# Alvin-Zeng/DRN

Measured on AMD Instinct MI355X. Metric: clips/sec fwd+bwd (BxT=256x4096 C3D feats), higher is better.
Workload: dtype bf16; 1 GPU; Charades-STA-shaped C3D features, T=256, D=4096, batch 32/GPU, stage-1 losses; step = fwd+bwd+grad all-reduce+clip(0.5)+Adam; global_batch=32, T=256, D=4096, parallelism=dp1

## Files before the change

drn_amd/csrc/api.hip:

```cpp
#include <stdarg.h>
#include "common.h"
#include "../../include/drn_hip.h"

static thread_local char g_err[512] = "";

void drn_set_error(const char* fmt, ...) {
  va_list ap;
  va_start(ap, fmt);
  vsnprintf(g_err, sizeof(g_err), fmt, ap);
  va_end(ap);
}

extern "C" int drn_abi_version(void) {
  drn_clear_status(); return DRN_ABI_VERSION; }
extern "C" const char* drn_last_error(void) { return g_err; }

static int g_tune[16] = {4096, 1, 256, 0, 0, 0, 0, 0, 1, 1, 0, 16, 160, 512, 2048, 1};
int drn_tuning(int key) { return g_tune[key]; }
extern "C" int drn_tune(const char* key, int value) {
  drn_clear_status();
  if (key && !strcmp(key, "tn3_minrows")) { g_tune[DRN_TUNE_TN3_MINROWS] = value; return DRN_OK; }
  if (key && !strcmp(key, "tn_fused")) { g_tune[DRN_TUNE_TN_FUSED] = value; return DRN_OK; }
  if (key && !strcmp(key, "nt_w4c")) { g_tune[DRN_TUNE_NT_W4C] = value; return DRN_OK; }
  if (key && !strcmp(key, "nt_w4")) { g_tune[DRN_TUNE_NT_W4] = value; return DRN_OK; }
  if (key && !strcmp(key, "nt_deep")) { g_tune[DRN_TUNE_NT_DEEP] = value; return DRN_OK; }
  if (key && !strcmp(key, "nt_w4h")) { g_tune[DRN_TUNE_NT_W4H] = value; return DRN_OK; }
  if (key && !strcmp(key, "w4h_tapil")) { g_tune[DRN_TUNE_W4H_TAPIL] = value; return DRN_OK; }
  if (key && !strcmp(key, "w4h_halo")) { g_tune[DRN_TUNE_W4H_HALO] = value; return DRN_OK; }
  if (key && !strcmp(key, "bn1_maxwg")) { g_tune[DRN_TUNE_BN1_MAXWG] = value; return DRN_OK; }
  if (key && !strcmp(key, "nt_deep2")) { g_tune[DRN_TUNE_NT_DEEP2] = value; return DRN_OK; }
  if (key && !strcmp(key, "nt_deep_ks")) { g_tune[DRN_TUNE_NT_DEEP_KS] = value; return DRN_OK; }
  if (key && !strncmp(key, "exp", 3) && key[3] >= '0' && key[3] <= '4' && !key[4]) { g_tune[DRN_TUNE_EXP0 + (key[3] - '0')] = value; return DRN_OK; }
  drn_set_error("drn_tune: unknown key %s", key ? key : "(null)");
  return DRN_ERR_ARG;
}
```

drn_amd/csrc/common.h:

```cpp
#pragma once
#include <hip/hip_runtime.h>
#include <stdint.h>
#include <stdio.h>
#include <string.h>

#define DRN_OK 0
#define DRN_ERR_ARG (-1)
#define DRN_ERR_LAUNCH (-2)
#define DRN_ERR_UNSUPPORTED (-3)

#define DRN_F32 0
#define DRN_BF16 1

typedef __bf16 bf16_t;
typedef __bf16 bf16x8 __attribute__((ext_vector_type(8)));
typedef __bf16 bf16x4 __attribute__((ext_vector_type(4)));
typedef short s16x4 __attribute__((ext_vector_type(4)));
typedef float f32x4 __attribute__((ext_vector_type(4)));
typedef float f32x2 __attribute__((ext_vector_type(2)));

template <typename T>
__device__ __forceinline__ T* as_global(T* p) {
  typedef __attribute__((address_space(1))) T* g_t;
  g_t g = (g_t)p;
  asm("" : "+s"(g));
  return (T*)g;
}
template <typename T>
__device__ __forceinline__ T* as_global_v(T* p) {
  typedef __attribute__((address_space(1))) T* g_t;
  g_t g = (g_t)p;
  asm("" : "+v"(g));
  return (T*)g;
}


void drn_set_error(const char* fmt, ...);

#define DRN_CHECK_ARG(cond, ...)          \
  do {                                    \
    if (!(cond)) {                        \
      drn_set_error(__VA_ARGS__);         \
      return DRN_ERR_ARG;                 \
    }                                     \
  } while (0)

static inline void drn_clear_status() { (void)hipGetLastError(); }

static inline int drn_launch_status(const char* what) {
  hipError_t e = hipGetLastError();
  if (e != hipSuccess) {
    drn_set_error("%s: launch failed: %s", what, hipGetErrorString(e));
    return DRN_ERR_LAUNCH;
  }
  return DRN_OK;
}

static inline int cdiv(int a, int b) { return (a + b - 1) / b; }

int drn_tuning(int key);
#define DRN_XCHG_CONFIRM 0x20000
#define DRN_XCHG_READBACK 0x40000
#define DRN_XCHG_NONE 0x80000
#define DRN_TUNE_TN3_MINROWS 0
#define DRN_TUNE_TN_FUSED 1
#define DRN_TUNE_EXP0 3
#define DRN_TUNE_NT_W4C 9
#define DRN_TUNE_NT_W4 8
#define DRN_TUNE_NT_DEEP 2
#define DRN_TUNE_NT_W4H 12
#define DRN_TUNE_BN1_MAXWG 13
#define DRN_TUNE_W4H_TAPIL 14
#define DRN_TUNE_W4H_HALO 15
#define DRN_TUNE_NT_DEEP2 10
#define DRN_TUNE_NT_DEEP_KS 11

static __device__ uint4 g_zero_page[4];

template <typename T> struct DT;
template <> struct DT<float> {
  static __device__ __forceinline__ float ld(const float* p) { return *p; }
  static __device__ __forceinline__ void st(float* p, float v) { *p = v; }
  static __device__ __forceinline__ float round(float v) { return v; }
};
template <> struct DT<bf16_t> {
  static __device__ __forceinline__ float ld(const bf16_t* p) { return (float)*p; }
  static __device__ __forceinline__ void st(bf16_t* p, float v) { *p = (bf16_t)v; }
  static __device__ __forceinline__ float round(float v) { return (float)(bf16_t)v; }
};

__device__ __forceinline__ float wave_sum(float v) {
#pragma unroll
  for (int o = 32; o > 0; o >>= 1) v += __shfl_xor(v, o, 64);
  return v;
}

__device__ __forceinline__ float block_sum(float v, float* sh ) {
  v = wave_sum(v);
  const int w = threadIdx.x >> 6, l = threadIdx.x & 63, nw = blockDim.x >> 6;
  __syncthreads();
  if (l == 0) sh[w] = v;
  __syncthreads();
  if (w == 0) {
    float t = l < nw ? sh[l] : 0.f;
    t = wave_sum(t);
    if (l == 0) sh[16] = t;
  }
  __syncthreads();
  return sh[16];
}
```

drn_amd/csrc/gemm_tn.hip:

```cpp
#include <type_traits>
#include "common.h"
#include "../../include/drn_hip.h"



struct WgradGroup {
  const void* dY;
  const void* X;
  int M, Lout, Lsrc, ldy, ldx;
  int blk_start;
};
struct WgradParams {
  int ngroups;
  WgradGroup g[DRN_MAX_GROUPS];
  int total_blks, blks_per_split;
  int N, Cin, taps, stride, pad;
  int ctiles;
  float* out;
  int direct;
  int w_layout;
  int accumulate;
  int multi;
  int z_start[DRN_MAX_GROUPS + 1], bps[DRN_MAX_GROUPS], gdirect[DRN_MAX_GROUPS];
  int gcin[DRN_MAX_GROUPS];
// ... 237 lines not shown
        if (c >= Cin) continue;
        float v = acc[mi][ni][r];
        if (direct) {
          float* dst = P.w_layout == 0 ? out_ptr + ((long)n * KW + tap * Cin + c)
                                       : out_ptr + ((long)n * KW + (long)c * P.taps + tap);
          if (P.accumulate) v += *dst;
          *dst = v;
        } else {
          out_ptr[((long)split * P.N + n) * KW + tap * Cin + c] = v;
        }
      }
    }
}

__device__ __forceinline__ bf16x8 tr_frag(const char* lo_addr, const char* hi_addr) {
  typedef __attribute__((address_space(3))) s16x4* lp;
  union { struct { s16x4 a, b; } s; bf16x8 v; } u;
  u.s.a = __builtin_amdgcn_ds_read_tr16_b64_v4i16((lp)lo_addr);
  u.s.b = __builtin_amdgcn_ds_read_tr16_b64_v4i16((lp)hi_addr);
  return u.v;
}

template <int NSTG>
__global__ __launch_bounds__(512, 2) void conv_wgrad3_tn_kernel(const WgradParams P) {
  extern __shared__ __attribute__((aligned(16))) char smem[];
  typedef bf16_t T;
  constexpr int R = 64, MI = 4, NI = 2;
  constexpr int IMG = 16384, HALO_B = 512, STAGE_B = 2 * IMG + HALO_B;
  const int tid = threadIdx.x, w = __builtin_amdgcn_readfirstlane(tid >> 6), l = tid & 63;
  const int n0 = blockIdx.x * 128, c0 = blockIdx.y * 128;
  int split = blockIdx.z;
  int blk_lo = split * P.blks_per_split;
  int blk_hi = min(blk_lo + P.blks_per_split, P.total_blks);
  float* out_ptr = P.out;
  int direct = P.direct;
  if (P.multi) {
    int pg = 0;
#pragma unroll
    for (int i = 1; i < DRN_MAX_GROUPS; ++i)
      if (i < P.ngroups && (int)blockIdx.z >= P.z_start[i]) pg = i;
    split = blockIdx.z - P.z_start[pg];
    const int blk_end = pg + 1 < P.ngroups ? P.g[pg + 1].blk_start : P.total_blks;
    blk_lo = P.g[pg].blk_start + split * P.bps[pg];
    blk_hi = min(blk_lo + P.bps[pg], blk_end);
    out_ptr = P.gout[pg];
    direct = P.gdirect[pg];
  }
  const T* zero = (const T*)g_zero_page;

  const int srow = w * 8 + (l >> 3);
  const int scol = (((l & 7) >> 1) ^ ((srow >> 1) & 3)) * 16 + (l & 1) * 8;
  long y_off[2], x_off[2];
#pragma unroll
  for (int j = 0; j < 2; ++j) {
    y_off[j] = n0 + j * 64 + scol < P.N ? n0 + j * 64 + scol : -1;
    x_off[j] = c0 + j * 64 + scol < P.Cin ? c0 + j * 64 + scol : -1;
  }
  const bool is_halo = (w == 0) & (l < 32);
  const int hcol = ((l >> 3) & 1) * 64 + (l & 7) * 8;
  const long xh_off = c0 + hcol < P.Cin ? c0 + hcol : -1;
  const int rowoff[2] = {srow, (l >> 4) ? R : -1};
  int s_blk = blk_lo, s_g = 0;
#pragma unroll
  for (int i = 1; i < DRN_MAX_GROUPS; ++i)
    if (i < P.ngroups && blk_lo >= P.g[i].blk_start) s_g = i;
  int s_seq[2], s_t[2];
  const T* g_Y;
  const T* g_X;
  int g_L, g_nseq, g_ldy, g_ldx, g_next;
  auto locate = [&]() {
    const WgradGroup& G = P.g[s_g];
    g_Y = (const T*)G.dY;
    g_X = (const T*)G.X;
    g_L = G.Lout;
    g_nseq = G.M / G.Lout;
    g_ldy = G.ldy;
    g_ldx = G.ldx;
    g_next = s_g + 1 < P.ngroups ? P.g[s_g + 1].blk_start : 0x7fffffff;
    const int Lp = G.Lout + 1;
    const int pbase = (s_blk - G.blk_start) * R;
#pragma unroll
    for (int j = 0; j < 2; ++j) {
      const int p = pbase + rowoff[j] + Lp;
      const int q = p / Lp;
      s_seq[j] = q - 1;
      s_t[j] = p - q * Lp;
    }
  };
  locate();

  auto row_ptr = [&](const T* base, int m, int ld, long coff, bool ok) -> const T* {
    const unsigned off = __umul24((unsigned)m, (unsigned)ld) + (unsigned)coff;
    const T* p = base + off;
    return ok ? p : zero;
  };
  auto stage_part = [&](int buf, int part) {
    char* Ys = smem + buf * STAGE_B;
    char* Xs = Ys + IMG;
    char* Hs = Xs + IMG;
    const bool live = s_blk < blk_hi;
    const int L = g_L;
    const bool ok = live & ((unsigned)s_seq[0] < (unsigned)g_nseq) & (s_t[0] < L);
    const int m = s_seq[0] * L + s_t[0];
    if (part == 0) glds16(row_ptr(g_Y, m, g_ldy, y_off[0], ok & (y_off[0] >= 0)), Ys + w * 1024);
    if (part == 1) glds16(row_ptr(g_X, m, g_ldx, x_off[0], ok & (x_off[0] >= 0)), Xs + w * 1024);
    if (part == 2) glds16(row_ptr(g_Y, m, g_ldy, y_off[1], ok & (y_off[1] >= 0)), Ys + 8192 + w * 1024);
    if (part == 3) {
      glds16(row_ptr(g_X, m, g_ldx, x_off[1], ok & (x_off[1] >= 0)), Xs + 8192 + w * 1024);
      if (is_halo) {
        const bool okh = live & ((unsigned)s_seq[1] < (unsigned)g_nseq) & (s_t[1] < L) & (xh_off >= 0);
        glds16(row_ptr(g_X, s_seq[1] * L + s_t[1], g_ldx, xh_off, okh), Hs);
      }
    }
    if (part != 4) return;
    ++s_blk;
    if (s_blk >= g_next) {
      ++s_g;
      locate();
    } else {
      const int Lp = L + 1;
      if (Lp > R) {
#pragma unroll
        for (int j = 0; j < 2; ++j) {
          s_t[j] += R;
          const bool wrap = s_t[j] >= Lp;
          s_t[j] -= wrap ? Lp : 0;
          s_seq[j] += wrap ? 1 : 0;
        }
      } else {
#pragma unroll
        for (int j = 0; j < 2; ++j) {
          s_t[j] += R;
          while (s_t[j] >= Lp) {
            s_t[j] -= Lp;
            ++s_seq[j];
          }
        }
      }
    }
  };
  auto stage = [&](int buf) {
#pragma unroll
    for (int part = 0; part < 5; ++part) stage_part(buf, part);
  };

  f32x4 acc[3][MI][NI];
#pragma unroll
  for (int t = 0; t < 3; ++t)
#pragma unroll
    for (int mi = 0; mi < MI; ++mi)
#pragma unroll
      for (int ni = 0; ni < NI; ++ni) acc[t][mi][ni] = (f32x4){0.f, 0.f, 0.f, 0.f};
  const int wr = w >> 2, wc = w & 3;

  const int fr = (l >> 4) * 4 + ((l & 15) >> 2);
  const int fb = (l & 3) * 8;
  int ya[MI], xa[3][NI], x_first[NI], x_last[NI];
#pragma unroll
  for (int mi = 0; mi < MI; ++mi) ya[mi] = wr * 8192 + fr * 128 + ((mi ^ ((fr >> 1) & 3)) * 32) + fb;
#pragma unroll
  for (int ni = 0; ni < NI; ++ni) {
    const int half = wc >> 1, cb = (wc & 1) * 2 + ni;
#pragma unroll
    for (int t = 0; t < 3; ++t) {
      const int rr = fr + t - 1;
      xa[t][ni] = IMG + half * 8192 + rr * 128 + ((cb ^ ((rr >> 1) & 3)) * 32) + fb;
    }
    x_first[ni] = fr == 0 ? 2 * IMG + half * 128 + cb * 32 + fb : xa[0][ni];
    x_last[ni] = fr == 15 ? 2 * IMG + 256 + half * 128 + cb * 32 + fb : xa[2][ni] + 4096 + 2048;
  }

  struct Frags {
    bf16x8 a[MI], b[3][NI];
  };
  auto load_frags = [&](Frags& F, const char* S, auto ks_) {
    constexpr int ks = decltype(ks_)::value;
#pragma unroll
    for (int mi = 0; mi < MI; ++mi) {
      const char* q = S + ya[mi] + ks * 4096;
      F.a[mi] = tr_frag(q, q + 2048);
    }
#pragma unroll
    for (int ni = 0; ni < NI; ++ni) {
      const char* q0 = S + xa[0][ni] + ks * 4096;
      const char* q1 = S + xa[1][ni] + ks * 4096;
      const char* q2 = S + xa[2][ni] + ks * 4096;
      F.b[1][ni] = tr_frag(q1, q1 + 2048);
      F.b[0][ni] = tr_frag(ks == 0 ? S + x_first[ni] : q0, q0 + 2048);
      F.b[2][ni] = tr_frag(q2, ks == 1 ? S + x_last[ni] : q2 + 2048);
    }
  };
  auto mfma_frags = [&](const Frags& F, int mi0) {
#pragma unroll
    for (int t = 0; t < 3; ++t)
#pragma unroll
      for (int mi = 0; mi < 2; ++mi)
#pragma unroll
        for (int ni = 0; ni < NI; ++ni)
          acc[t][mi0 + mi][ni] = __builtin_amdgcn_mfma_f32_16x16x32_bf16(F.a[mi0 + mi], F.b[t][ni], acc[t][mi0 + mi][ni], 0, 0, 0);
  };
  typedef std::integral_constant<int, 0> K0;
  typedef std::integral_constant<int, 1> K1;

  auto wait_landed = [&](int younger) {
    if (younger <= 0) asm volatile("s_waitcnt vmcnt(0)" ::: "memory");
    else if (younger == 1) { if (w == 0) asm volatile("s_waitcnt vmcnt(5)" ::: "memory"); else asm volatile("s_waitcnt vmcnt(4)" ::: "memory"); }
    else { if (w == 0) asm volatile("s_waitcnt vmcnt(10)" ::: "memory"); else asm volatile("s_waitcnt vmcnt(8)" ::: "memory"); }
  };
#pragma unroll
  for (int st = 0; st < NSTG - 1; ++st) stage(st);
  wait_landed(NSTG - 2);
  __builtin_amdgcn_s_barrier();
  asm volatile("" ::: "memory");
  Frags F0, F1;
  load_frags(F0, smem, K0());
  int cur = 0;
  for (int blk = blk_lo; blk < blk_hi; ++blk) {
    wait_landed(NSTG - 3);
    __builtin_amdgcn_s_barrier();
    asm volatile("" ::: "memory");
    int nxt = cur + NSTG - 1;
    if (nxt >= NSTG) nxt -= NSTG;
    const int cn = cur + 1 == NSTG ? 0 : cur + 1;
    load_frags(F1, smem + cur * STAGE_B, K1());
    stage_part(nxt, 0);
    __builtin_amdgcn_sched_barrier(0);
    mfma_frags(F0, 0);
    __builtin_amdgcn_sched_barrier(0);
    stage_part(nxt, 1);
    __builtin_amdgcn_sched_barrier(0);
    mfma_frags(F0, 2);
    __builtin_amdgcn_sched_barrier(0);
    load_frags(F0, smem + cn * STAGE_B, K0());
    stage_part(nxt, 2);
    __builtin_amdgcn_sched_barrier(0);
    mfma_frags(F1, 0);
    __builtin_amdgcn_sched_barrier(0);
    stage_part(nxt, 3);
    __builtin_amdgcn_sched_barrier(0);
    mfma_frags(F1, 2);
    __builtin_amdgcn_sched_barrier(0);
    stage_part(nxt, 4);
    cur = cn;
  }
  asm volatile("s_waitcnt vmcnt(0)" ::: "memory");

  const int KW = 3 * P.Cin;
  const bool rowmajor = !direct || (P.w_layout == 0 && !P.accumulate);
  float* obase = direct ? out_ptr : out_ptr + (long)split * P.N * KW;
  if (rowmajor && (P.Cin % 4 == 0) && (((uintptr_t)obase & 15) == 0)) {
    constexpr int PITCH = 32 * 4 + 16;
    __syncthreads();
    char* wbuf = smem + w * (32 * PITCH);
#pragma unroll
    for (int t = 0; t < 3; ++t)
#pragma unroll
      for (int ch = 0; ch < MI / 2; ++ch) {
        const int nrow0 = n0 + wr * 64 + ch * 32;
#pragma unroll
        for (int mi2 = 0; mi2 < 2; ++mi2)
#pragma unroll
          for (int r = 0; r < 4; ++r)
#pragma unroll
            for (int ni = 0; ni < NI; ++ni)
              *((float*)(wbuf + (mi2 * 16 + (l >> 4) * 4 + r) * PITCH) + ni * 16 + (l & 15)) = acc[t][ch * 2 + mi2][ni][r];
        asm volatile("s_waitcnt lgkmcnt(0)" ::: "memory");
#pragma unroll
        for (int it = 0; it < 4; ++it) {
          const int rl = it * 8 + (l >> 3), cv = l & 7;
          const int n = nrow0 + rl, c = c0 + wc * 32 + cv * 4;
          if (n < P.N && c < P.Cin) {
            const f32x4 v = *(const f32x4*)(wbuf + rl * PITCH + cv * 16);
            *(f32x4*)(obase + ((long)n * KW + t * P.Cin + c)) = v;
          }
        }
        asm volatile("s_waitcnt lgkmcnt(0)" ::: "memory");
      }
    return;
  }
#pragma unroll
  for (int t = 0; t < 3; ++t)
#pragma unroll
    for (int mi = 0; mi < MI; ++mi)
#pragma unroll
      for (int r = 0; r < 4; ++r) {
        const int n = n0 + wr * 64 + mi * 16 + (l >> 4) * 4 + r;
        if (n >= P.N) continue;
#pragma unroll
        for (int ni = 0; ni < NI; ++ni) {
          const int c = c0 + wc * 32 + ni * 16 + (l & 15);
          if (c >= P.Cin) continue;
          float v = acc[t][mi][ni][r];
          if (direct) {
            float* dst = P.w_layout == 0 ? out_ptr + ((long)n * KW + t * P.Cin + c) : out_ptr + ((long)n * KW + (long)c * 3 + t);
            if (P.accumulate) v += *dst;
            *dst = v;
          } else {
            out_ptr[((long)split * P.N + n) * KW + t * P.Cin + c] = v;
          }
        }
      }
}

struct WgradReduceMulti {
  const float* ws[DRN_MAX_GROUPS];
  float* out[DRN_MAX_GROUPS];
  int nsplit[DRN_MAX_GROUPS];
  int cin[DRN_MAX_GROUPS];
};
__global__ void wgrad_reduce_multi_kernel(const WgradReduceMulti R, int N, int taps, int w_layout, int accumulate) {
  const int Cin = R.cin[blockIdx.y];
  const long KW = (long)taps * Cin;
  const long total = (long)N * KW;
  const float* __restrict__ ws = R.ws[blockIdx.y];
  float* __restrict__ out = R.out[blockIdx.y];
  const int nsplit = R.nsplit[blockIdx.y];
  if (nsplit <= 1) return;
  if (w_layout == 1 && taps == 3) {
    const long pairs = (long)N * Cin;
    for (long idx = (long)blockIdx.x * blockDim.x + threadIdx.x; idx < pairs; idx += (long)gridDim.x * blockDim.x) {
      const long n = idx / Cin;
      const int c = (int)(idx - n * Cin);
      const float* p = ws + n * KW + c;
      float s0 = 0.f, s1 = 0.f, s2 = 0.f;
#pragma unroll 4
      for (int z = 0; z < nsplit; ++z) {
        s0 += p[(long)z * total];
        s1 += p[(long)z * total + Cin];
        s2 += p[(long)z * total + 2 * Cin];
      }
      float* o = out + n * KW + (long)c * 3;
      if (accumulate) {
        s0 += o[0];
        s1 += o[1];
        s2 += o[2];
      }
      o[0] = s0;
      o[1] = s1;
      o[2] = s2;
    }
    return;
  }
  for (long idx = (long)blockIdx.x * blockDim.x + threadIdx.x; idx < total; idx += (long)gridDim.x * blockDim.x) {
    float s = 0.f;
    for (int z = 0; z < nsplit; ++z) s += ws[(long)z * total + idx];
    long o = idx;
    if (w_layout == 1) {
      const long n = idx / KW;
      const int rem = (int)(idx - n * KW);
      const int tap = rem / Cin, c = rem - tap * Cin;
      o = n * KW + (long)c * taps + tap;
    }
    if (accumulate) s += out[o];
    out[o] = s;
  }
}

__global__ void wgrad_reduce_kernel(const float* __restrict__ ws, float* __restrict__ out, int nsplit, int N, int Cin,
                                    int taps, int w_layout, int accumulate) {
  const long KW = (long)taps * Cin;
  const long total = (long)N * KW;
  if (w_layout == 1 && taps == 3) {
    const long pairs = (long)N * Cin;
    for (long idx = (long)blockIdx.x * blockDim.x + threadIdx.x; idx < pairs; idx += (long)gridDim.x * blockDim.x) {
      const long n = idx / Cin;
      const int c = (int)(idx - n * Cin);
      const float* p = ws + n * KW + c;
      float s0 = 0.f, s1 = 0.f, s2 = 0.f;
#pragma unroll 4
      for (int z = 0; z < nsplit; ++z) {
        s0 += p[(long)z * total];
        s1 += p[(long)z * total + Cin];
        s2 += p[(long)z * total + 2 * Cin];
      }
      float* o = out + n * KW + (long)c * 3;
      if (accumulate) {
        s0 += o[0];
        s1 += o[1];
        s2 += o[2];
      }
      o[0] = s0;
      o[1] = s1;
      o[2] = s2;
    }
    return;
  }
  for (long idx = (long)blockIdx.x * blockDim.x + threadIdx.x; idx < total; idx += (long)gridDim.x * blockDim.x) {
    float s = 0.f;
    for (int z = 0; z < nsplit; ++z) s += ws[(long)z * total + idx];
    long o = idx;
    if (w_layout == 1) {
      const long n = idx / KW;
      const int rem = (int)(idx - n * KW);
      const int tap = rem / Cin, c = rem - tap * Cin;
      o = n * KW + (long)c * taps + tap;
    }
    if (accumulate) s += out[o];
    out[o] = s;
  }
}

typedef DrnWgradPendItem WgradPendItem;
#define WGRAD_PEND_MAX DRN_WGRAD_PEND_MAX
typedef DrnWgradPending WgradPendParams;

static int wgrad_pend_push(DrnWgradPending* L, const float* ws, float* out, int nsplit, int N, int Cin, int taps, int w_layout, int accumulate) {
  if (!L || L->n < 0 || L->n >= WGRAD_PEND_MAX) return 0;
  for (int i = 0; i < L->n; ++i)
    if (L->it[i].out == out) {
      drn_set_error("drn_gemm_wgrad: the output already has a deferred reduce pending in this DrnWgradPending (flush with drn_wgrad_reduce_pending first)");
      return DRN_ERR_ARG;
    }
  if (accumulate) return 0;
  L->it[L->n++] = WgradPendItem{ws, out, nsplit, N, Cin, taps, w_layout, accumulate};
  return 1;
}

__global__ __launch_bounds__(256) void wgrad_reduce_all_kernel(const WgradPendParams P) {
  __shared__ float sh_sq[17];
  float sq = 0.f;
  int i = 0;
  for (int k = 1; k < P.n; ++k)
    if ((int)blockIdx.x >= P.blk_start[k]) i = k;
  const WgradPendItem& I = P.it[i];
  const int nb = P.blk_start[i + 1] - P.blk_start[i], b = blockIdx.x - P.blk_start[i];
  const float* __restrict__ ws = I.ws;
  float* __restrict__ out = I.out;
  const int N = I.N, Cin = I.Cin, taps = I.taps, nsplit = I.nsplit, accumulate = I.accumulate, w_layout = I.w_layout;
  const long KW = (long)taps * Cin;
  const long total = (long)N * KW;
  if (w_layout == 1 && taps == 3) {
    const long pairs = (long)N * Cin;
    for (long idx = (long)b * 256 + threadIdx.x; idx < pairs; idx += (long)nb * 256) {
      const long n = idx / Cin;
      const int c = (int)(idx - n * Cin);
      const float* p = ws + n * KW + c;
      float s0 = 0.f, s1 = 0.f, s2 = 0.f;
#pragma unroll 4
      for (int z = 0; z < nsplit; ++z) {
        s0 += __builtin_nontemporal_load(p + (long)z * total);
        s1 += __builtin_nontemporal_load(p + (long)z * total + Cin);
        s2 += __builtin_nontemporal_load(p + (long)z * total + 2 * Cin);
      }
      float* o = out + n * KW + (long)c * 3;
      if (accumulate) {
        s0 += o[0];
        s1 += o[1];
        s2 += o[2];
      }
      o[0] = s0;
      o[1] = s1;
      o[2] = s2;
      sq = fmaf(s0, s0, sq); sq = fmaf(s1, s1, sq); sq = fmaf(s2, s2, sq);
    }
  } else {
    for (long idx = (long)b * 256 + threadIdx.x; idx < total; idx += (long)nb * 256) {
      float s = 0.f;
      for (int z = 0; z < nsplit; ++z) s += __builtin_nontemporal_load(ws + (long)z * total + idx);
      long o = idx;
      if (w_layout == 1) {
        const long n = idx / KW;
        const int rem = (int)(idx - n * KW);
        const int tap = rem / Cin, c = rem - tap * Cin;
        o = n * KW + (long)c * taps + tap;
      }
      if (accumulate) s += out[o];
      out[o] = s;
      sq = fmaf(s, s, sq);
    }
  }
  if (P.sumsq) {
    sq = block_sum(sq, sh_sq);
    if (threadIdx.x == 0) P.sumsq[blockIdx.x] = sq;
  }
}

static int wgrad_pend_plan(DrnWgradPending* L) {
  int blocks = 0;
  for (int i = 0; i < L->n; ++i) {
    const WgradPendItem& I = L->it[i];
    const long work = (I.w_layout == 1 && I.taps == 3) ? (long)I.N * I.Cin : (long)I.N * I.taps * I.Cin;
    int nb = (int)((work + 255) / 256);
    if (nb > 2048) nb = 2048;
    L->blk_start[i] = blocks;
    blocks += nb;
  }
  L->blk_start[L->n] = blocks;
  return blocks;
}

extern "C" int drn_wgrad_pending_blocks(DrnWgradPending* L) {
  drn_clear_status();
  DRN_CHECK_ARG(L && L->n >= 0 && L->n <= WGRAD_PEND_MAX, "drn_wgrad_pending_blocks: bad list");
  return wgrad_pend_plan(L);
}

extern "C" int64_t drn_wgrad_pending_bytes(const DrnWgradPending* L) {
  int64_t b = 0;
  if (!L || L->n < 0 || L->n > WGRAD_PEND_MAX) return 0;
  for (int i = 0; i < L->n; ++i) {
    const WgradPendItem& I = L->it[i];
    b += (int64_t)I.N * I.taps * I.Cin * 4 * (I.nsplit + 1 + (I.accumulate ? 1 : 0));
  }
  return b;
}

extern "C" int drn_wgrad_reduce_pending(DrnWgradPending* L, float* sumsq, void* stream) {
  drn_clear_status();
  DRN_CHECK_ARG(L && L->n >= 0 && L->n <= WGRAD_PEND_MAX, "drn_wgrad_reduce_pending: bad list");
  if (L->n == 0) return DRN_OK;
  const int blocks = wgrad_pend_plan(L);
  L->sumsq = sumsq;
  wgrad_reduce_all_kernel<<<blocks, 256, 0, (hipStream_t)stream>>>(*L);
  L->n = 0;
  L->sumsq = nullptr;
  return drn_launch_status("drn_wgrad_reduce_pending");
}

static int wgrad_tile(int N, int Cin, int taps) {
  return (long)cdiv(N, 256) * taps * cdiv(Cin, 256) >= 128 ? 256 : 128;
}

static int wgrad_nsplit(int total_blks, int N, int Cin, int taps) {
  const int tile = wgrad_tile(N, Cin, taps);
  const int tiles = cdiv(N, tile) * taps * cdiv(Cin, tile);
  const int tgt = drn_tuning(DRN_TUNE_EXP0 + 2) > 0 ? drn_tuning(DRN_TUNE_EXP0 + 2) : 768;
  int ns = cdiv(tile == 256 ? 256 : tgt, tiles);
  const int cap = total_blks / 12;
  if (ns > cap) ns = cap;
  if (ns < 1) ns = 1;
  if (ns > 64) ns = 64;
  return ns;
}

static int total_blocks_upper(int M_total, int ngroups_max) {
  return cdiv(M_total, 32) + ngroups_max;
}

static int wgrad3_nsplit(int m_total, int N, int Cin) {
  const int target = drn_tuning(DRN_TUNE_EXP0 + 1) > 0 ? drn_tuning(DRN_TUNE_EXP0 + 1) : 256;
  const int tiles = cdiv(N, 128) * cdiv(Cin, 128);
  int ns = target / tiles;
  const int cap = cdiv(m_total, 64) / 8;
  if (ns > cap) ns = cap;
  if (ns < 1) ns = 1;
  if (ns > 64) ns = 64;
  return ns;
}
static bool wgrad3_enabled() {
  return drn_tuning(DRN_TUNE_TN_FUSED) != 0;
}
static bool wgrad3_group_ok(const DrnWgradDesc& s) {
  return s.Lsrc == s.Lout && s.M < (1 << 24) && s.ldy < (1 << 24) && s.ldx < (1 << 24) &&
         (long)s.M * s.ldy < (1L << 31) && (long)s.M * s.ldx < (1L << 31);
}
static int wgrad3_min_rows() {
  return drn_tuning(DRN_TUNE_TN3_MINROWS);
}
static void wgrad3_attr() {
  static bool set = false;
  if (!set) {
    (void)hipFuncSetAttribute((const void*)conv_wgrad3_tn_kernel<4>, hipFuncAttributeMaxDynamicSharedMemorySize, 163840);
    set = true;
  }
}
#define WGRAD3_STAGE (2 * 16384 + 512)
#define WGRAD3_LAUNCH(GRID, P) conv_wgrad3_tn_kernel<4><<<GRID, 512, 4 * WGRAD3_STAGE, stream>>>(P)

extern "C" int64_t drn_wgrad_ws_elems(int M_total, int N, int Cin, int taps) {
  int ns = wgrad_nsplit(total_blocks_upper(M_total, DRN_MAX_GROUPS), N, Cin, taps);
  if (taps == 3) {
    const int ns3 = wgrad3_nsplit(M_total, N, Cin);
    if (ns3 > ns) ns = ns3;
  }
  return ns > 1 ? (int64_t)ns * N * taps * Cin : 0;
}

extern "C" int drn_gemm_wgrad(const DrnWgradDesc* d, int ngroups, float* dW, int N, int Cin, int taps, int stride, int pad,
                              int w_layout, int accumulate, float* ws, int dtype, DrnWgradPending* pend, void* stream_) {
  drn_clear_status();
  hipStream_t stream = (hipStream_t)stream_;
  DRN_CHECK_ARG(ngroups >= 1 && ngroups <= DRN_MAX_GROUPS, "drn_gemm_wgrad: ngroups=%d out of range", ngroups);
  DRN_CHECK_ARG(dtype == DRN_F32 || dtype == DRN_BF16, "drn_gemm_wgrad: bad dtype %d", dtype);
  DRN_CHECK_ARG(dW && N > 0 && Cin > 0 && taps >= 1 && stride >= 1, "drn_gemm_wgrad: bad dims");
  if (pend)
    for (int i = 0; i < pend->n && i < WGRAD_PEND_MAX; ++i)
      DRN_CHECK_ARG(pend->it[i].out != dW, "drn_gemm_wgrad: the output already has a deferred reduce pending in this DrnWgradPending (flush first)");
  const int ch = dtype == DRN_BF16 ? 8 : 4;
  const int R = dtype == DRN_BF16 ? 64 : 32;
  WgradParams P;
  memset(&P, 0, sizeof(P));
  P.ngroups = ngroups;
  int blks = 0, m_total = 0;
  for (int g = 0; g < ngroups; ++g) {
    const DrnWgradDesc& s = d[g];
    DRN_CHECK_ARG(s.dY && s.X && s.M > 0 && s.Lout > 0 && s.Lsrc > 0 && s.M % s.Lout == 0, "drn_gemm_wgrad: bad group %d", g);
    DRN_CHECK_ARG(s.ldy % ch == 0 && s.ldx % ch == 0 && N % ch == 0 && Cin % ch == 0,
                  "drn_gemm_wgrad: N/Cin/ldy/ldx must be multiples of %d elements", ch);
    DRN_CHECK_ARG(((uintptr_t)s.dY & 15) == 0 && ((uintptr_t)s.X & 15) == 0, "drn_gemm_wgrad: operands must be 16-byte aligned");
    P.g[g].dY = s.dY; P.g[g].X = s.X; P.g[g].M = s.M; P.g[g].Lout = s.Lout; P.g[g].Lsrc = s.Lsrc;
    P.g[g].ldy = s.ldy; P.g[g].ldx = s.ldx; P.g[g].blk_start = blks;
    blks += cdiv(s.M, R);
    m_total += s.M;
  }
  bool fused = dtype == DRN_BF16 && taps == 3 && stride == 1 && pad == 1 && wgrad3_enabled() && m_total >= wgrad3_min_rows();
  for (int g = 0; g < ngroups; ++g) fused = fused && wgrad3_group_ok(d[g]);
  if (fused) {
    blks = 0;
    for (int g = 0; g < ngroups; ++g) {
      P.g[g].blk_start = blks;
      blks += cdiv((d[g].M / d[g].Lout) * (d[g].Lout + 1), 64);
    }
    int ns = wgrad3_nsplit(m_total, N, Cin);
    if (ns > blks) ns = blks;
    DRN_CHECK_ARG(ns == 1 || ws, "drn_gemm_wgrad: workspace required (drn_wgrad_ws_elems)");
    P.total_blks = blks;
    P.blks_per_split = cdiv(blks, ns);
    ns = cdiv(blks, P.blks_per_split);
    P.N = N; P.Cin = Cin; P.taps = taps; P.stride = stride; P.pad = pad;
    P.ctiles = cdiv(Cin, 128);
    P.direct = ns == 1;
    P.out = P.direct ? dW : ws;
    P.w_layout = w_layout;
    P.accumulate = accumulate;
    wgrad3_attr();
    WGRAD3_LAUNCH(dim3(cdiv(N, 128), cdiv(Cin, 128), ns), P);
    int rc = drn_launch_status("drn_gemm_wgrad(fused taps)");
    if (rc) return rc;
    const int pushed = P.direct ? 0 : wgrad_pend_push(pend, ws, dW, ns, N, Cin, taps, w_layout, accumulate);
    if (pushed < 0) return pushed;
    if (!P.direct && !pushed) {
      const long total = (long)N * taps * Cin;
      int nb = (int)((total + 255) / 256);
      if (nb > 2048) nb = 2048;
      wgrad_reduce_kernel<<<nb, 256, 0, stream>>>(ws, dW, ns, N, Cin, taps, w_layout, accumulate);
      rc = drn_launch_status("drn_gemm_wgrad(reduce)");
    }
    return rc;
  }
  int ns = wgrad_nsplit(total_blocks_upper(m_total, DRN_MAX_GROUPS), N, Cin, taps);
  if (ns > blks) ns = blks;
  DRN_CHECK_ARG(ns == 1 || ws, "drn_gemm_wgrad: workspace required (drn_wgrad_ws_elems)");
  P.total_blks = blks;
  P.blks_per_split = cdiv(blks, ns);
  ns = cdiv(blks, P.blks_per_split);
  P.N = N; P.Cin = Cin; P.taps = taps; P.stride = stride; P.pad = pad;
  const int tile = wgrad_tile(N, Cin, taps);
  P.ctiles = cdiv(Cin, tile);
  P.direct = ns == 1;
  P.out = P.direct ? dW : ws;
  P.w_layout = w_layout;
  P.accumulate = accumulate;
  static bool attr_set = false;
  if (!attr_set) {
    (void)hipFuncSetAttribute((const void*)conv_wgrad_tn_kernel<float, 2, 2, 4, 4>, hipFuncAttributeMaxDynamicSharedMemorySize, 163840);
    (void)hipFuncSetAttribute((const void*)conv_wgrad_tn_kernel<bf16_t, 2, 2, 4, 4>, hipFuncAttributeMaxDynamicSharedMemorySize, 163840);
    (void)hipFuncSetAttribute((const void*)conv_wgrad_tn_kernel<float, 2, 4, 8, 4>, hipFuncAttributeMaxDynamicSharedMemorySize, 163840);
    (void)hipFuncSetAttribute((const void*)conv_wgrad_tn_kernel<bf16_t, 2, 4, 8, 4>, hipFuncAttributeMaxDynamicSharedMemorySize, 163840);
    (void)hipFuncSetAttribute((const void*)conv_wgrad_tn_kernel<float, 2, 4, 4, 2>, hipFuncAttributeMaxDynamicSharedMemorySize, 163840);
    (void)hipFuncSetAttribute((const void*)conv_wgrad_tn_kernel<bf16_t, 2, 4, 4, 2>, hipFuncAttributeMaxDynamicSharedMemorySize, 163840);
    attr_set = true;
  }
  dim3 grid(cdiv(N, tile), taps * P.ctiles, ns);
  if (tile == 256) {
    if (dtype == DRN_BF16) conv_wgrad_tn_kernel<bf16_t, 2, 4, 8, 4><<<grid, 512, 2 * 65536, stream>>>(P);
    else conv_wgrad_tn_kernel<float, 2, 4, 8, 4><<<grid, 512, 2 * 65536, stream>>>(P);
  } else {
    if (dtype == DRN_BF16) conv_wgrad_tn_kernel<bf16_t, 2, 4, 4, 2><<<grid, 512, 2 * 32768, stream>>>(P);
    else conv_wgrad_tn_kernel<float, 2, 4, 4, 2><<<grid, 512, 2 * 32768, stream>>>(P);
  }
  int rc = drn_launch_status("drn_gemm_wgrad");
  if (rc) return rc;
  const int pushed = P.direct ? 0 : wgrad_pend_push(pend, ws, dW, ns, N, Cin, taps, w_layout, accumulate);
  if (pushed < 0) return pushed;
  if (!P.direct && !pushed) {
    const long total = (long)N * taps * Cin;
    int nb = (int)((total + 255) / 256);
    if (nb > 2048) nb = 2048;
    wgrad_reduce_kernel<<<nb, 256, 0, stream>>>(ws, dW, ns, N, Cin, taps, w_layout, accumulate);
    rc = drn_launch_status("drn_gemm_wgrad(reduce)");
  }
  return rc;
}

extern "C" int drn_gemm_wgrad_multi(const DrnWgradDesc* d, int n, float* const* dWs, int N, int Cin, const int32_t* Cins, int taps,
                                    int stride, int pad, int w_layout, int accumulate, float* ws, int dtype, DrnWgradPending* pend,
                                    void* stream_) {
  drn_clear_status();
  hipStream_t stream = (hipStream_t)stream_;
  DRN_CHECK_ARG(d && dWs && n >= 1 && n <= DRN_MAX_GROUPS, "drn_gemm_wgrad_multi: n=%d out of range", n);
  if (pend)
    for (int g = 0; g < n; ++g)
      for (int i = 0; i < pend->n && i < WGRAD_PEND_MAX; ++i)
        DRN_CHECK_ARG(pend->it[i].out != dWs[g], "drn_gemm_wgrad_multi: output %d already has a deferred reduce pending in this DrnWgradPending", g);
  DRN_CHECK_ARG(dtype == DRN_F32 || dtype == DRN_BF16, "drn_gemm_wgrad_multi: bad dtype %d", dtype);
  DRN_CHECK_ARG(N > 0 && Cin > 0 && taps >= 1 && stride >= 1, "drn_gemm_wgrad_multi: bad dims");
  const int ch = dtype == DRN_BF16 ? 8 : 4;
  const int R = dtype == DRN_BF16 ? 64 : 32;
  const int tile = 128;
  WgradParams P;
  WgradReduceMulti RM;
  memset(&P, 0, sizeof(P));
  memset(&RM, 0, sizeof(RM));
  P.ngroups = n;
  P.multi = 1;
  bool varied = false;
  for (int g = 0; g < n && Cins; ++g) {
    DRN_CHECK_ARG(Cins[g] > 0 && Cins[g] <= Cin && Cins[g] % ch == 0, "drn_gemm_wgrad_multi: bad Cins[%d]", g);
    varied |= Cins[g] != Cin;
  }
  int blks = 0, z = 0, mmax = 0;
  bool any_split = false;
  for (int g = 0; g < n; ++g) mmax = d[g].M > mmax ? d[g].M : mmax;
  const long ws_per = drn_wgrad_ws_elems(mmax, N, Cin, taps);
  bool fused = !varied && dtype == DRN_BF16 && taps == 3 && stride == 1 && pad == 1 && wgrad3_enabled() && mmax >= wgrad3_min_rows();
  for (int g = 0; g < n; ++g) fused = fused && wgrad3_group_ok(d[g]);
  for (int g = 0; g < n; ++g) {
    const DrnWgradDesc& s = d[g];
    DRN_CHECK_ARG(s.dY && s.X && dWs[g] && s.M > 0 && s.Lout > 0 && s.Lsrc > 0 && s.M % s.Lout == 0, "drn_gemm_wgrad_multi: bad problem %d", g);
    DRN_CHECK_ARG(s.ldy % ch == 0 && s.ldx % ch == 0 && N % ch == 0 && Cin % ch == 0,
                  "drn_gemm_wgrad_multi: N/Cin/ldy/ldx must be multiples of %d elements", ch);
    DRN_CHECK_ARG(((uintptr_t)s.dY & 15) == 0 && ((uintptr_t)s.X & 15) == 0, "drn_gemm_wgrad_multi: operands must be 16-byte aligned");
    P.g[g].dY = s.dY; P.g[g].X = s.X; P.g[g].M = s.M; P.g[g].Lout = s.Lout; P.g[g].Lsrc = s.Lsrc;
    P.g[g].ldy = s.ldy; P.g[g].ldx = s.ldx; P.g[g].blk_start = blks;
    const int gb = fused ? cdiv((s.M / s.Lout) * (s.Lout + 1), 64) : cdiv(s.M, R);
    blks += gb;
    const int cin_g = Cins ? Cins[g] : Cin;
    const long per = (long)N * taps * cin_g;
    P.gcin[g] = cin_g; RM.cin[g] = cin_g;
    int ns = wgrad_nsplit(total_blocks_upper(s.M, 1), N, cin_g, taps);
    if (fused) {
      long m_all = 0;
      for (int k = 0; k < n; ++k) m_all += d[k].M;
      ns = (int)((long)wgrad3_nsplit(mmax, N, Cin) * s.M / m_all);
      const int cap = gb / 4;
      if (ns > cap) ns = cap;
      if (ns < 1) ns = 1;
    }
    if (ns > gb) ns = gb;
    P.bps[g] = cdiv(gb, ns);
    ns = cdiv(gb, P.bps[g]);
    DRN_CHECK_ARG(ns == 1 || ws, "drn_gemm_wgrad_multi: workspace required");
    P.z_start[g] = z;
    z += ns;
    P.gdirect[g] = ns == 1;
    P.gout[g] = ns == 1 ? dWs[g] : ws + (long)g * ws_per;
    RM.ws[g] = ws + (long)g * ws_per; RM.out[g] = dWs[g]; RM.nsplit[g] = ns;
    any_split |= ns > 1;
    DRN_CHECK_ARG(ns == 1 || (long)ns * per <= ws_per, "drn_gemm_wgrad_multi: workspace slice too small");
  }
  P.z_start[n] = z;
  P.total_blks = blks;
  P.blks_per_split = blks;
  P.N = N; P.Cin = Cin; P.taps = taps; P.stride = stride; P.pad = pad;
  P.ctiles = cdiv(Cin, tile);
  P.w_layout = w_layout;
  P.accumulate = accumulate;
  static bool attr_set = false;
  if (!attr_set) {
    (void)hipFuncSetAttribute((const void*)conv_wgrad_tn_kernel<float, 2, 4, 4, 2>, hipFuncAttributeMaxDynamicSharedMemorySize, 163840);
    (void)hipFuncSetAttribute((const void*)conv_wgrad_tn_kernel<bf16_t, 2, 4, 4, 2>, hipFuncAttributeMaxDynamicSharedMemorySize, 163840);
    attr_set = true;
  }
  dim3 grid(cdiv(N, tile), taps * P.ctiles, z);
  if (fused) {
    wgrad3_attr();
    WGRAD3_LAUNCH(dim3(cdiv(N, 128), cdiv(Cin, 128), z), P);
  } else if (dtype == DRN_BF16) conv_wgrad_tn_kernel<bf16_t, 2, 4, 4, 2><<<grid, 512, 2 * 32768, stream>>>(P);
  else conv_wgrad_tn_kernel<float, 2, 4, 4, 2><<<grid, 512, 2 * 32768, stream>>>(P);
  int rc = drn_launch_status("drn_gemm_wgrad_multi");
  if (rc || !any_split) return rc;
  if (pend && !accumulate && pend->n >= 0 && pend->n + n <= WGRAD_PEND_MAX) {
    for (int g = 0; g < n; ++g)
      if (RM.nsplit[g] > 1) (void)wgrad_pend_push(pend, RM.ws[g], RM.out[g], RM.nsplit[g], N, RM.cin[g], taps, w_layout, accumulate);
    return rc;
  }
  int nb = (int)(((long)N * taps * Cin + 255) / 256);
  if (nb > 1024) nb = 1024;
  wgrad_reduce_multi_kernel<<<dim3(nb, n), 256, 0, stream>>>(RM, N, taps, w_layout, accumulate);
  return drn_launch_status("drn_gemm_wgrad_multi(reduce)");
}
```

Baseline: 17380 clips/s.

## Add warp-specialized producer/consumer wgrad3 kernel with dedicated load waves

```diff
diff --git a/drn_amd/csrc/api.hip b/drn_amd/csrc/api.hip
--- a/drn_amd/csrc/api.hip
+++ b/drn_amd/csrc/api.hip
@@ -15,12 +15,17 @@
   drn_clear_status(); return DRN_ABI_VERSION; }
 extern "C" const char* drn_last_error(void) { return g_err; }
 
-static int g_tune[16] = {4096, 1, 256, 0, 0, 0, 0, 0, 1, 1, 0, 16, 160, 512, 2048, 1};
+static int g_tune[16] = {4096, 1 | (1 << DRN_TUNE_TN3_ROLES_SHIFT), 256, 0, 0, 0, 0, 0, 1, 1, 0, 16, 160, 512, 2048, 1};
 int drn_tuning(int key) { return g_tune[key]; }
 extern "C" int drn_tune(const char* key, int value) {
   drn_clear_status();
   if (key && !strcmp(key, "tn3_minrows")) { g_tune[DRN_TUNE_TN3_MINROWS] = value; return DRN_OK; }
-  if (key && !strcmp(key, "tn_fused")) { g_tune[DRN_TUNE_TN_FUSED] = value; return DRN_OK; }
+  if (key && !strcmp(key, "tn_fused")) { g_tune[DRN_TUNE_TN_FUSED] = (g_tune[DRN_TUNE_TN_FUSED] & ~0xff) | (value != 0); return DRN_OK; }
+  if (key && !strcmp(key, "tn3_roles")) {
+    if (value < 0 || value > 5) { drn_set_error("drn_tune: tn3_roles=%d out of range (0..5)", value); return DRN_ERR_ARG; }
+    g_tune[DRN_TUNE_TN_FUSED] = (g_tune[DRN_TUNE_TN_FUSED] & 0xff) | (value << DRN_TUNE_TN3_ROLES_SHIFT);
+    return DRN_OK;
+  }
   if (key && !strcmp(key, "nt_w4c")) { g_tune[DRN_TUNE_NT_W4C] = value; return DRN_OK; }
   if (key && !strcmp(key, "nt_w4")) { g_tune[DRN_TUNE_NT_W4] = value; return DRN_OK; }
   if (key && !strcmp(key, "nt_deep")) { g_tune[DRN_TUNE_NT_DEEP] = value; return DRN_OK; }
diff --git a/drn_amd/csrc/common.h b/drn_amd/csrc/common.h
--- a/drn_amd/csrc/common.h
+++ b/drn_amd/csrc/common.h
@@ -64,6 +64,7 @@
 #define DRN_XCHG_NONE 0x80000
 #define DRN_TUNE_TN3_MINROWS 0
 #define DRN_TUNE_TN_FUSED 1
+#define DRN_TUNE_TN3_ROLES_SHIFT 8
 #define DRN_TUNE_EXP0 3
 #define DRN_TUNE_NT_W4C 9
 #define DRN_TUNE_NT_W4 8
diff --git a/drn_amd/csrc/gemm_tn.hip b/drn_amd/csrc/gemm_tn.hip
--- a/drn_amd/csrc/gemm_tn.hip
+++ b/drn_amd/csrc/gemm_tn.hip
@@ -563,6 +563,287 @@
       }
 }
 
+template <int NP>
+__global__ __launch_bounds__(512 + 64 * NP) void conv_wgrad3_roles_kernel(const WgradParams P) {
+  extern __shared__ __attribute__((aligned(16))) char smem[];
+  typedef bf16_t T;
+  constexpr int R = 64, MI = 4, NI = 2, NSTG = 4;
+  constexpr int IMG = 16384, HALO_B = 512, STAGE_B = 2 * IMG + HALO_B;
+  constexpr int KP = 8 / NP;
+  constexpr int YOUNG = NP >= 2 ? 2 : 1;
+  static_assert(NP == 1 || NP == 2 || NP == 4, "one, two or four producer waves");
+  static_assert(YOUNG * (KP * 4 + 1) <= 63, "vmcnt is a 6-bit counter");
+  const int tid = threadIdx.x, w = __builtin_amdgcn_readfirstlane(tid >> 6), l = tid & 63;
+  const int n0 = blockIdx.x * 128, c0 = blockIdx.y * 128;
+  int split = blockIdx.z;
+  int blk_lo = split * P.blks_per_split;
+  int blk_hi = min(blk_lo + P.blks_per_split, P.total_blks);
+  float* out_ptr = P.out;
+  int direct = P.direct;
+  if (P.multi) {
+    int pg = 0;
+#pragma unroll
+    for (int i = 1; i < DRN_MAX_GROUPS; ++i)
+      if (i < P.ngroups && (int)blockIdx.z >= P.z_start[i]) pg = i;
+    split = blockIdx.z - P.z_start[pg];
+    const int blk_end = pg + 1 < P.ngroups ? P.g[pg + 1].blk_start : P.total_blks;
+    blk_lo = P.g[pg].blk_start + split * P.bps[pg];
+    blk_hi = min(blk_lo + P.bps[pg], blk_end);
+    out_ptr = P.gout[pg];
+    direct = P.gdirect[pg];
+  }
+
+  if (w >= 8) {
+#ifdef WGRAD3R_PRIO
+    __builtin_amdgcn_s_setprio(WGRAD3R_PRIO);
+#endif
+    const int pw = w - 8;
+    const T* zero = (const T*)g_zero_page;
+    const int lrow = l >> 3;
+    const int scol = (((l & 7) >> 1) ^ ((lrow >> 1) & 3)) * 16 + (l & 1) * 8;
+    long y_off[2], x_off[2];
+#pragma unroll
+    for (int j = 0; j < 2; ++j) {
+      y_off[j] = n0 + j * 64 + scol < P.N ? n0 + j * 64 + scol : -1;
+      x_off[j] = c0 + j * 64 + scol < P.Cin ? c0 + j * 64 + scol : -1;
+    }
+    const bool is_halo = (pw == 0) & (l < 32);
+    const int hcol = ((l >> 3) & 1) * 64 + (l & 7) * 8;
+    const long xh_off = c0 + hcol < P.Cin ? c0 + hcol : -1;
+    int rowoff[KP + 1];
+#pragma unroll
+    for (int i = 0; i < KP; ++i) rowoff[i] = (pw * KP + i) * 8 + lrow;
+    rowoff[KP] = (l >> 4) ? R : -1;
+    int s_blk = blk_lo, s_g = 0;
+#pragma unroll
+    for (int i = 1; i < DRN_MAX_GROUPS; ++i)
+      if (i < P.ngroups && blk_lo >= P.g[i].blk_start) s_g = i;
+    int s_seq[KP + 1], s_t[KP + 1];
+    const T* g_Y;
+    const T* g_X;
+    int g_L, g_nseq, g_ldy, g_ldx, g_next;
+    auto locate = [&]() {
+      const WgradGroup& G = P.g[s_g];
+      g_Y = (const T*)G.dY;
+      g_X = (const T*)G.X;
+      g_L = G.Lout;
+      g_nseq = G.M / G.Lout;
+      g_ldy = G.ldy;
+      g_ldx = G.ldx;
+      g_next = s_g + 1 < P.ngroups ? P.g[s_g + 1].blk_start : 0x7fffffff;
+      const int Lp = G.Lout + 1;
+      const int pbase = (s_blk - G.blk_start) * R;
+#pragma unroll
+      for (int j = 0; j < KP + 1; ++j) {
+        const int p = pbase + rowoff[j] + Lp;
+        const int q = p / Lp;
+        s_seq[j] = q - 1;
+        s_t[j] = p - q * Lp;
+      }
+    };
+    locate();
+    auto row_ptr = [&](const T* base, int m, int ld, long coff, bool ok) -> const T* {
+      const unsigned off = __umul24((unsigned)m, (unsigned)ld) + (unsigned)coff;
+      const T* p = base + off;
+      return ok ? p : zero;
+    };
+    auto stage = [&](int buf) {
+      char* Ys = smem + buf * STAGE_B;
+      char* Xs = Ys + IMG;
+      char* Hs = Xs + IMG;
+      const bool live = s_blk < blk_hi;
+      const int L = g_L;
+#ifndef WGRAD3R_NO_STAGE
+#pragma unroll
+      for (int i = 0; i < KP; ++i) {
+        const int k = pw * KP + i;
+        const bool ok = live & ((unsigned)s_seq[i] < (unsigned)g_nseq) & (s_t[i] < L);
+        const int m = s_seq[i] * L + s_t[i];
+        glds16(row_ptr(g_Y, m, g_ldy, y_off[0], ok & (y_off[0] >= 0)), Ys + k * 1024);
+        glds16(row_ptr(g_X, m, g_ldx, x_off[0], ok & (x_off[0] >= 0)), Xs + k * 1024);
+        glds16(row_ptr(g_Y, m, g_ldy, y_off[1], ok & (y_off[1] >= 0)), Ys + 8192 + k * 1024);
+        glds16(row_ptr(g_X, m, g_ldx, x_off[1], ok & (x_off[1] >= 0)), Xs + 8192 + k * 1024);
+      }
+      if (is_halo) {
+        const bool okh = live & ((unsigned)s_seq[KP] < (unsigned)g_nseq) & (s_t[KP] < L) & (xh_off >= 0);
+        glds16(row_ptr(g_X, s_seq[KP] * L + s_t[KP], g_ldx, xh_off, okh), Hs);
+      }
+#endif
+      ++s_blk;
+      if (s_blk >= g_next) {
+        ++s_g;
+        locate();
+      } else {
+        const int Lp = L + 1;
+        if (Lp > R) {
+#pragma unroll
+          for (int j = 0; j < KP + 1; ++j) {
+            s_t[j] += R;
+            const bool wrap = s_t[j] >= Lp;
+            s_t[j] -= wrap ? Lp : 0;
+            s_seq[j] += wrap ? 1 : 0;
+          }
+        } else {
+#pragma unroll
+          for (int j = 0; j < KP + 1; ++j) {
+            s_t[j] += R;
+            while (s_t[j] >= Lp) {
+              s_t[j] -= Lp;
+              ++s_seq[j];
+            }
+          }
+        }
+      }
+    };
+#pragma unroll
+    for (int st = 0; st < NSTG - 1; ++st) stage(st);
+    int nxt = NSTG - 1;
+    for (int blk = blk_lo; blk < blk_hi; ++blk) {
+#ifndef WGRAD3R_NO_STAGE
+      if (pw == 0) asm volatile("s_waitcnt vmcnt(%0)" ::"n"(YOUNG * (KP * 4 + 1)) : "memory");
+      else asm volatile("s_waitcnt vmcnt(%0)" ::"n"(YOUNG * (KP * 4)) : "memory");
+#endif
+      __builtin_amdgcn_s_barrier();
+      asm volatile("" ::: "memory");
+      stage(nxt);
+      nxt = nxt + 1 == NSTG ? 0 : nxt + 1;
+    }
+    asm volatile("s_waitcnt vmcnt(0)" ::: "memory");
+    __builtin_amdgcn_s_barrier();
+    return;
+  }
+
+  f32x4 acc[3][MI][NI];
+#pragma unroll
+  for (int t = 0; t < 3; ++t)
+#pragma unroll
+    for (int mi = 0; mi < MI; ++mi)
+#pragma unroll
+      for (int ni = 0; ni < NI; ++ni) acc[t][mi][ni] = (f32x4){0.f, 0.f, 0.f, 0.f};
+  const int wr = w >> 2, wc = w & 3;
+  {
+    const int fr = (l >> 4) * 4 + ((l & 15) >> 2);
+    const int fb = (l & 3) * 8;
+    int ya[MI], xa[3][NI], x_first[NI], x_last[NI];
+#pragma unroll
+    for (int mi = 0; mi < MI; ++mi) ya[mi] = wr * 8192 + fr * 128 + ((mi ^ ((fr >> 1) & 3)) * 32) + fb;
+#pragma unroll
+    for (int ni = 0; ni < NI; ++ni) {
+      const int half = wc >> 1, cb = (wc & 1) * 2 + ni;
+#pragma unroll
+      for (int t = 0; t < 3; ++t) {
+        const int rr = fr + t - 1;
+        xa[t][ni] = IMG + half * 8192 + rr * 128 + ((cb ^ ((rr >> 1) & 3)) * 32) + fb;
+      }
+      x_first[ni] = fr == 0 ? 2 * IMG + half * 128 + cb * 32 + fb : xa[0][ni];
+      x_last[ni] = fr == 15 ? 2 * IMG + 256 + half * 128 + cb * 32 + fb : xa[2][ni] + 4096 + 2048;
+    }
+    struct Frags {
+      bf16x8 a[MI], b[3][NI];
+    };
+    auto load_frags = [&](Frags& F, const char* S, auto ks_) {
+      constexpr int ks = decltype(ks_)::value;
+#pragma unroll
+      for (int mi = 0; mi < MI; ++mi) {
+        const char* q = S + ya[mi] + ks * 4096;
+        F.a[mi] = tr_frag(q, q + 2048);
+      }
+#pragma unroll
+      for (int ni = 0; ni < NI; ++ni) {
+        const char* q0 = S + xa[0][ni] + ks * 4096;
+        const char* q1 = S + xa[1][ni] + ks * 4096;
+        const char* q2 = S + xa[2][ni] + ks * 4096;
+        F.b[1][ni] = tr_frag(q1, q1 + 2048);
+        F.b[0][ni] = tr_frag(ks == 0 ? S + x_first[ni] : q0, q0 + 2048);
+        F.b[2][ni] = tr_frag(q2, ks == 1 ? S + x_last[ni] : q2 + 2048);
+      }
+    };
+    auto mfma_frags = [&](const Frags& F, int mi0) {
+#pragma unroll
+      for (int t = 0; t < 3; ++t)
+#pragma unroll
+        for (int mi = 0; mi < 2; ++mi)
+#pragma unroll
+          for (int ni = 0; ni < NI; ++ni)
+            acc[t][mi0 + mi][ni] = __builtin_amdgcn_mfma_f32_16x16x32_bf16(F.a[mi0 + mi], F.b[t][ni], acc[t][mi0 + mi][ni], 0, 0, 0);
+    };
+    typedef std::integral_constant<int, 0> K0;
+    typedef std::integral_constant<int, 1> K1;
+    int cur = 0;
+    for (int blk = blk_lo; blk < blk_hi; ++blk) {
+      __builtin_amdgcn_s_barrier();
+      asm volatile("" ::: "memory");
+#ifndef WGRAD3R_NO_MFMA
+      const char* S = smem + cur * STAGE_B;
+      Frags F;
+      load_frags(F, S, K0());
+      mfma_frags(F, 0);
+      mfma_frags(F, 2);
+      load_frags(F, S, K1());
+      mfma_frags(F, 0);
+      mfma_frags(F, 2);
+#endif
+      cur = cur + 1 == NSTG ? 0 : cur + 1;
+    }
+  }
+  __syncthreads();
+
+  const int KW = 3 * P.Cin;
+  const bool rowmajor = !direct || (P.w_layout == 0 && !P.accumulate);
+  float* obase = direct ? out_ptr : out_ptr + (long)split * P.N * KW;
+  if (rowmajor && (P.Cin % 4 == 0) && (((uintptr_t)obase & 15) == 0)) {
+    constexpr int PITCH = 32 * 4 + 16;
+    char* wbuf = smem + w * (32 * PITCH);
+#pragma unroll
+    for (int t = 0; t < 3; ++t)
+#pragma unroll
+      for (int ch = 0; ch < MI / 2; ++ch) {
+        const int nrow0 = n0 + wr * 64 + ch * 32;
+#pragma unroll
+        for (int mi2 = 0; mi2 < 2; ++mi2)
+#pragma unroll
+          for (int r = 0; r < 4; ++r)
+#pragma unroll
+            for (int ni = 0; ni < NI; ++ni)
+              *((float*)(wbuf + (mi2 * 16 + (l >> 4) * 4 + r) * PITCH) + ni * 16 + (l & 15)) = acc[t][ch * 2 + mi2][ni][r];
+        asm volatile("s_waitcnt lgkmcnt(0)" ::: "memory");
+#pragma unroll
+        for (int it = 0; it < 4; ++it) {
+          const int rl = it * 8 + (l >> 3), cv = l & 7;
+          const int n = nrow0 + rl, c = c0 + wc * 32 + cv * 4;
+          if (n < P.N && c < P.Cin) {
+            const f32x4 v = *(const f32x4*)(wbuf + rl * PITCH + cv * 16);
+            *(f32x4*)(obase + ((long)n * KW + t * P.Cin + c)) = v;
+          }
+        }
+        asm volatile("s_waitcnt lgkmcnt(0)" ::: "memory");
+      }
+    return;
+  }
+#pragma unroll
+  for (int t = 0; t < 3; ++t)
+#pragma unroll
+    for (int mi = 0; mi < MI; ++mi)
+#pragma unroll
+      for (int r = 0; r < 4; ++r) {
+        const int n = n0 + wr * 64 + mi * 16 + (l >> 4) * 4 + r;
+        if (n >= P.N) continue;
+#pragma unroll
+        for (int ni = 0; ni < NI; ++ni) {
+          const int c = c0 + wc * 32 + ni * 16 + (l & 15);
+          if (c >= P.Cin) continue;
+          float v = acc[t][mi][ni][r];
+          if (direct) {
+            float* dst = P.w_layout == 0 ? out_ptr + ((long)n * KW + t * P.Cin + c) : out_ptr + ((long)n * KW + (long)c * 3 + t);
+            if (P.accumulate) v += *dst;
+            *dst = v;
+          } else {
+            out_ptr[((long)split * P.N + n) * KW + t * P.Cin + c] = v;
+          }
+        }
+      }
+}
+
 struct WgradReduceMulti {
   const float* ws[DRN_MAX_GROUPS];
   float* out[DRN_MAX_GROUPS];
@@ -809,7 +1090,14 @@
   return ns;
 }
 static bool wgrad3_enabled() {
-  return drn_tuning(DRN_TUNE_TN_FUSED) != 0;
+  return (drn_tuning(DRN_TUNE_TN_FUSED) & 0xff) != 0;
+}
+#define WGRAD3_PRODUCERS 4
+static int wgrad3_roles(int blks_per_split) {
+  const int mode = drn_tuning(DRN_TUNE_TN_FUSED) >> DRN_TUNE_TN3_ROLES_SHIFT;
+  if (mode >= 3) return 1 << (mode - 3);
+  if (mode == 2) return WGRAD3_PRODUCERS;
+  return mode == 1 && blks_per_split >= 8 ? WGRAD3_PRODUCERS : 0;
 }
 static bool wgrad3_group_ok(const DrnWgradDesc& s) {
   return s.Lsrc == s.Lout && s.M < (1 << 24) && s.ldy < (1 << 24) && s.ldx < (1 << 24) &&
@@ -822,11 +1110,20 @@
   static bool set = false;
   if (!set) {
     (void)hipFuncSetAttribute((const void*)conv_wgrad3_tn_kernel<4>, hipFuncAttributeMaxDynamicSharedMemorySize, 163840);
+    (void)hipFuncSetAttribute((const void*)conv_wgrad3_roles_kernel<2>, hipFuncAttributeMaxDynamicSharedMemorySize, 163840);
+    (void)hipFuncSetAttribute((const void*)conv_wgrad3_roles_kernel<1>, hipFuncAttributeMaxDynamicSharedMemorySize, 163840);
+    (void)hipFuncSetAttribute((const void*)conv_wgrad3_roles_kernel<4>, hipFuncAttributeMaxDynamicSharedMemorySize, 163840);
     set = true;
   }
 }
 #define WGRAD3_STAGE (2 * 16384 + 512)
-#define WGRAD3_LAUNCH(GRID, P) conv_wgrad3_tn_kernel<4><<<GRID, 512, 4 * WGRAD3_STAGE, stream>>>(P)
+#define WGRAD3_LAUNCH(GRID, P, ROLES)                                                                          \
+  do {                                                                                                         \
+    if ((ROLES) == 4) conv_wgrad3_roles_kernel<4><<<GRID, 768, 4 * WGRAD3_STAGE, stream>>>(P);                  \
+    else if ((ROLES) == 2) conv_wgrad3_roles_kernel<2><<<GRID, 640, 4 * WGRAD3_STAGE, stream>>>(P);             \
+    else if ((ROLES) == 1) conv_wgrad3_roles_kernel<1><<<GRID, 576, 4 * WGRAD3_STAGE, stream>>>(P);             \
+    else conv_wgrad3_tn_kernel<4><<<GRID, 512, 4 * WGRAD3_STAGE, stream>>>(P);                                 \
+  } while (0)
 
 extern "C" int64_t drn_wgrad_ws_elems(int M_total, int N, int Cin, int taps) {
   int ns = wgrad_nsplit(total_blocks_upper(M_total, DRN_MAX_GROUPS), N, Cin, taps);
@@ -885,7 +1182,7 @@
     P.w_layout = w_layout;
     P.accumulate = accumulate;
     wgrad3_attr();
-    WGRAD3_LAUNCH(dim3(cdiv(N, 128), cdiv(Cin, 128), ns), P);
+    WGRAD3_LAUNCH(dim3(cdiv(N, 128), cdiv(Cin, 128), ns), P, wgrad3_roles(P.blks_per_split));
     int rc = drn_launch_status("drn_gemm_wgrad(fused taps)");
     if (rc) return rc;
     const int pushed = P.direct ? 0 : wgrad_pend_push(pend, ws, dW, ns, N, Cin, taps, w_layout, accumulate);
@@ -1026,7 +1323,9 @@
   dim3 grid(cdiv(N, tile), taps * P.ctiles, z);
   if (fused) {
     wgrad3_attr();
-    WGRAD3_LAUNCH(dim3(cdiv(N, 128), cdiv(Cin, 128), z), P);
+    int bps_min = P.bps[0];
+    for (int g = 1; g < n; ++g) bps_min = P.bps[g] < bps_min ? P.bps[g] : bps_min;
+    WGRAD3_LAUNCH(dim3(cdiv(N, 128), cdiv(Cin, 128), z), P, wgrad3_roles(bps_min));
   } else if (dtype == DRN_BF16) conv_wgrad_tn_kernel<bf16_t, 2, 4, 4, 2><<<grid, 512, 2 * 32768, stream>>>(P);
   else conv_wgrad_tn_kernel<float, 2, 4, 4, 2><<<grid, 512, 2 * 32768, stream>>>(P);
   int rc = drn_launch_status("drn_gemm_wgrad_multi");
```

Result: no change. 17480 clips/s, median of 6 (+0.5%).
